# Somedaywilldo/BM-NAS

Measured on AMD Instinct MI355X. Metric: search-steps/sec (fwd+bwd of fusion hypernet) on MM-IMDB synthetic, higher is better.
Workload: dtype f32; 1 GPU; mmimdb fusion search, batch 128 per GPU x 1 GPU(s), N6 C192 L16 steps2 node_steps1 node_multiplier1, train mode, dropout 0.1/0.1(attn); inputs=(b, C, L) features, global_batch=128, per_gpu_batch=128, parallelism=dp1, mode=graph, step=fwd+bwd, one hipGraph replay

## Files before the change

### bm-nas_amd/bmnas/cell.py

```python
from __future__ import annotations

import os

import torch

from . import lib

ATTN_DROP = 0.1

OVERLAP = False
_SIDE = {}


class _Fork:

    def __init__(self, device):
        self.main = torch.cuda.current_stream(device)
        if OVERLAP:
            key = (device.index, self.main.cuda_stream)
            s = _SIDE.get(key)
            if s is None:
                s = torch.cuda.Stream(device)
                _SIDE[key] = s
            self.stream = s
# ... 309 lines not shown
    sv.stats1 = _empty(x, b * 2)
    sv.p1 = p1
    sv.d_glu = DROP.make(P.glu_p, x.numel(), training)
    sv.d_fc = DROP.make(P.fc_p, x.numel(), training)
    sv.merged = same and FUSE_ATTN_GEMM
    if sv.merged:
        U, chan = _mixed_conv_fwd(sv, x, y, same, P, training, C,
                                  attn=(x, y, P.ln_w, P.ln_b, p1, sv.xhat1, sv.stats1, C, sv.d_attn), Weff=Weff,
                                  stats=stats)
    else:
        with _Fork(x.device) as fork:
            fork.side(lambda: lib.sdpa_ln_fwd(x, y, P.ln_w, P.ln_b, p1, sv.xhat1, sv.stats1, b, C, L, sv.d_attn))
            U, chan = _mixed_conv_fwd(sv, x, y, same, P, training, C, Weff=Weff, stats=stats)
    out = torch.empty_like(x)
    fin = sv.conv.fin
    if not launch_mix:
        sv.pending_mix = (x, y, p1, U, chan, gamma_row, out, sv.d_glu, sv.d_fc, fin)
        return out, sv
    if ln is None:
        lib.node_mix_fwd(x, y, p1, U, chan, gamma_row, out, b, C, L, sv.d_glu, sv.d_fc, fin, nxt)
    else:
        resid, ln_w, ln_b, ln_stats, out_sums, lazy = ln
        sv.pre = torch.empty_like(x)
        if lazy:
            P = lib.lazy_ln_parts(C, L)
            rec, prm = _empty(x, b * P * 8), _empty(x, P * 8)
            lib.node_mix_pre_fwd(x, y, p1, U, chan, gamma_row, resid, ln_w, ln_b, sv.pre, rec, prm, b, C, L,
                                 sv.d_glu, sv.d_fc, fin)
            sv.lazy = LazyNode(desc=lib.make_lazy(sv.pre, rec, prm, ln_w, ln_b, ln_stats), out=out, P=P,
                               rec=rec, prm=prm)
        else:
            lib.node_mix_ln_fwd(x, y, p1, U, chan, gamma_row, resid, ln_w, ln_b, sv.pre, out, ln_stats, b, C, L,
                                sv.d_glu, sv.d_fc, fin, out_sums)
    return out, sv


FUSE_ATTN_GEMM = os.environ.get('BMNAS_FUSE_ATTN_GEMM', '1') != '0'
FUSE_PROLOGUE = os.environ.get('BMNAS_FUSE_PROLOGUE', '1') != '0'
FUSE_EPILOGUE = os.environ.get('BMNAS_FUSE_EPILOGUE', '1') != '0'
FUSE_BN_FINALIZE = os.environ.get('BMNAS_FUSE_BN_FINALIZE', '1') != '0'
FUSE_BN_APPLY = os.environ.get('BMNAS_FUSE_BN_APPLY', '1') != '0'
FUSE_MIX_GEMM = os.environ.get('BMNAS_FUSE_MIX_GEMM', '1') != '0'
FUSE_BWD_PAIR = os.environ.get('BMNAS_FUSE_BWD_PAIR', '1') != '0'
FUSE_BN_TAIL = os.environ.get('BMNAS_FUSE_BN_TAIL', '1') != '0'
BN_TAIL_MAX_B = 128
FUSE_INNER_SUM = os.environ.get('BMNAS_FUSE_INNER_SUM', '1') != '0'
MIX_PREV_MAX = 5
FUSE_PROLOGUE_PAIR = os.environ.get('BMNAS_FUSE_PROLOGUE_PAIR', '1') != '0'
FUSE_LN_BWD = os.environ.get('BMNAS_FUSE_LN_BWD', '1') != '0'
FUSE_NEXT_PAIR = os.environ.get('BMNAS_FUSE_NEXT_PAIR', '1') != '0'
FUSE_MIX_EPILOGUE = os.environ.get('BMNAS_FUSE_MIX_EPILOGUE', '1') != '0'
FUSE_HEAD = os.environ.get('BMNAS_FUSE_HEAD', '1') != '0'
LAZY_LN = os.environ.get('BMNAS_LAZY_LN', '1') != '0'
WRITE_ONCE = os.environ.get('BMNAS_WRITE_ONCE', '1') != '0'


STRICT_ZERO = os.environ.get('BMNAS_STRICT_ZERO', '0') not in ('0', '', 'false', 'False')


DETERMINISTIC = os.environ.get('BMNAS_DETERMINISTIC', '0') not in ('0', '', 'false', 'False')
_DET_APPLIED = [None]


def apply_deterministic():
    if _DET_APPLIED[0] != DETERMINISTIC:
        lib.set_deterministic(DETERMINISTIC)
        _DET_APPLIED[0] = DETERMINISTIC


def arch_shards(b, C, L):
    if not DETERMINISTIC:
        return ARCH_SHARDS
    cl4 = C * L // 4
    parts = (cl4 + 255) // 256
    streaming = min(2048, (b * cl4 + 255) // 256)
    mix = ((cl4 + 63) // 64) * lib.node_mix_lnp_bwd_rows(b)
    return max(ARCH_SHARDS, b * parts, streaming, mix)


class LazyNode(Pack):
    materialised = False
    lnp_head = None
    lnp_k1 = None
    k1_n = 0


def _mixed_conv_fwd(sv, x, y, same, P, training, C, attn=None, Weff=None, stats=None):
    if same:
        if Weff is None:
            M = P.stack_W.shape[0]
            Weff = _empty(x, M, C)
            lib.fold_weight(P.stack_W, Weff, M, C)
        U, chan, sv.conv = conv_bn_fwd([x], C, Weff, C, P.stack_bias, P.stack_bn_w, P.stack_bn_b,
                                       P.stack_rm, P.stack_rv, P.stack_nbt, training, dup=C, attn=attn,
                                       stats=stats)
    else:
        U, chan, sv.conv = conv_bn_fwd([x, y], C, P.stack_W, 2 * C, P.stack_bias, P.stack_bn_w,
                                       P.stack_bn_b, P.stack_rm, P.stack_rv, P.stack_nbt, training,
                                       stats=stats)
    return U, chan


class Deferred:

# ... 375 lines not shown

def fusion_cell_fwd(xs, alpha_w, beta_ws, gamma_ws, CP, training, S, M, ns, nm, weffs=None, stats=None,
                    head=None, prologue=None):
    N = len(xs)
    b, C, L = xs[0].shape
    sv = CellSaved()
    sv.N, sv.S, sv.M, sv.CP, sv.alpha_w = N, S, M, CP, alpha_w
    states = list(xs)
    sv.sifs, sv.nodes, sv.offsets = [], [], []
    offset = 0
    pending_pair = None
    sv.lazy_on = bool(LAZY_LN and head is not None and nm == 1 and FUSE_TAIL and FUSE_PAIR and N + S <= 15
                      and 1 <= S <= 3 and M <= S and (C * L) % 64 == 0 and xs[0].is_cuda and lib.lazy_ln_ok(C, L))
    for i in range(S):
        if pending_pair is not None:
            sif, z0 = pending_pair
            pending_pair = None
        elif FUSE_PAIR and len(states) <= 15:
            sif, z0 = torch.empty_like(xs[0]), torch.empty_like(xs[0])
            lz = sv.nodes[-1].lazy if (sv.lazy_on and i >= 1) else None
            if i == 0 and prologue is not None:
                prologue(states, sif, z0)
            elif lz is not None and not lz.materialised:
                lib.mixsum_pair_fwd_lazy(states[:-1], alpha_w[offset:, 1], 2, beta_ws[i][:, 1], 2, lz.desc,
                                         states[-1], sv.nodes[-1].osum, sif, z0, b, C, L)
                lz.materialised = True
            else:
                lib.mixsum_pair_fwd(states, alpha_w[offset:, 1], 2, beta_ws[i][:, 1], 2, sif, z0)
        else:
            sif, z0 = mixsum_fwd(states, alpha_w[offset:, 1]), None
        if STRICT_ZERO:
            if i == 0:
                poison = xs[0] * 0.
                for x_ in xs[1:]:
                    poison = poison + x_ * 0.
            sif.add_(poison)
            if z0 is not None:
                z0.add_(poison)
        next_pair = None
        if (FUSE_NEXT_PAIR and FUSE_PAIR and FUSE_BN_TAIL and i + 1 < S and nm != 1 and len(states) + 1 <= 15
                and lib.bn_relu_ln_fwd_pair_ok(b, C, L, len(states))):
            nsif, nz0 = torch.empty_like(xs[0]), torch.empty_like(xs[0])
            next_pair = (list(states), alpha_w[offset + len(states):, 1], 2, beta_ws[i + 1][:, 1], 2, nsif, nz0)
        out, nsv = node_cell_fwd(sif, sif, beta_ws[i], gamma_ws[i], CP.nodes[i], training, ns, nm, z0,
                                 None if weffs is None else weffs[i * ns:(i + 1) * ns], stats,
                                 want_sums=head is not None, next_pair=next_pair, lazy=sv.lazy_on)
        if next_pair is not None and nsv.next_pair_done:
            pending_pair = (next_pair[5], next_pair[6])
        nsv.paired = z0 is not None
        sv.sifs.append(sif)
        sv.nodes.append(nsv)
        sv.offsets.append(offset)
        offset += len(states)
        states.append(out)
    sv.states = states
    sv.stats = _empty(xs[0], b * 2)
    sv.head = head
    if head is not None:
        if M > S:
            raise lib.BmnasError('fused head: the cell concatenates input states (multiplier > steps)')
        head.sums = [nsv.osum for nsv in sv.nodes[S - M:]]
        if DETERMINISTIC and (not sv.lazy_on or ns != 1):
            raise lib.BmnasError('BMNAS_DETERMINISTIC covers the search cell with node_steps == 1 and node_multiplier '
                                 '== 1 under the fused head (the lazy-LayerNorm path); this configuration is outside it')
        last = sv.nodes[-1].lazy if sv.lazy_on else None
        if last is not None and not last.materialised:
            O_ = head.W.shape[0]
            hb_part = _empty(xs[0], lib.head_fwd_part_floats(b, C, L, M, O_)) if DETERMINISTIC else None
            lib.head_fwd_lazy(states[-M:-1] + [sv.nodes[-1].o], head.sums[:-1] + [None], M - 1, last.desc, CP.ln_w,
# ... 162 lines not shown
```

### bm-nas_amd/bmnas/lib.py

```python
import ctypes as C
import os

import torch

HERE = os.path.dirname(os.path.abspath(__file__))
LIB_PATH = os.environ.get('BMNAS_LIB') or os.path.join(HERE, 'libbmnas_hip.so')
MAX_PTRS = 16


class BmnasError(RuntimeError):
    pass


_NOTED = set()


def note_off_path(where, why):
    key = (where, why)
    if key not in _NOTED:
        _NOTED.add(key)
        import warnings
        warnings.warn(f'bmnas: {where} runs on the stock torch ops, not the HIP kernels: {why}', RuntimeWarning,
                      stacklevel=3)

# ... 205 lines not shown
    'bmnas_unroll_virtual_step': ([_P, _P, _I, _P, _I, _P], _I),
    'bmnas_unroll_perturb': ([_P, _P, _I, _P, _I, _P, C.c_float, _P, _P], _I),
    'bmnas_unroll_restore': ([_P, _P, _I, _P], _I),
    'bmnas_unroll_combine': ([_P, _P, _I, _P, _P, _P], _I),
    'bmnas_copy_batch_max': ([], _I),
    'bmnas_copy_blob_max': ([], _I),
    'bmnas_copy_batch': ([_PP, _PP, C.POINTER(C.c_longlong), _I, _P, _P, _I, _P, C.c_ulonglong, _P], _I),
    'bmnas_arch_softmax_fwd': ([_P, _P, _I, _I, _P], _I),
    'bmnas_arch_softmax_bwd': ([_P, _P, _P, _I, _I, _P], _I),
    'bmnas_backward_epilogue': ([_I, _PP, _PP, C.POINTER(_PP), C.POINTER(C.c_int), _PP, _PP, _PP, _PP, _PP,
                                 _PP, _I, C.POINTER(C.c_int), _I, C.POINTER(C.c_int), C.POINTER(C.c_int),
                                 _PP, _PP, _PP, C.POINTER(C.c_int), C.POINTER(C.c_int), _I, _I, _I64,
                                 _I, _PP, _PP, C.POINTER(C.c_int), C.POINTER(C.c_int64), _P], _I),
    'bmnas_head_chunks': ([_I], _I),
    'bmnas_head_fwd': ([_PP, _PP, _I, _P, _P, _P, _P, _P, _P, _I, _I, _I, _I, _P], _I),
    'bmnas_debug_stamps': ([_P, _I], _I),
    'bmnas_debug_stamps_head': ([_P, _I], _I),
    'bmnas_debug_stamps_conv': ([_P, _I], _I),
    'bmnas_lazy_ln_ok': ([_I, _I], _I),
    'bmnas_lazy_ln_parts': ([_I, _I], _I),
    'bmnas_node_mix_pre_fwd': ([_P, _P, _P, _P, _P, BnFin, _P, _P, _P, _P, _P, _P, _P, _I, _I, _I, Dropout, Dropout,
                                _P], _I),
    'bmnas_mixsum_pair_fwd_lazy': ([_PP, _I, _P, _I, _P, _I, C.POINTER(LazyLn), _P, _P, _P, _P, _I, _I, _I, _P], _I),
    'bmnas_mixsum_pair_bwd_lazy': ([_PP, _PP, _I, _P, _I, _P, _I, _P, _P, _P, _P, _P, _P, _I, _I64, _U32,
                                    C.POINTER(LazyLn), _PP, C.POINTER(C.c_int), _I, _P, _I, _I, _I, _P], _I),
    'bmnas_mixsum_pair_bwd_x': ([_PP, _PP, _I, _P, _I, _P, _I, _P, _P, _P, _P, _P, _P, _I, _I64, _U32, _PP, _PP, _I,
                                 _I64, _P], _I),
    'bmnas_head_fwd_lazy': ([_PP, _PP, _I, _I, C.POINTER(LazyLn), _P, _P, _P, _P, _P, _P, _I, _I, _I, _I, _P, _P], _I),
    'bmnas_head_fwd_part_floats': ([_I, _I, _I, _I, _I], _I),
    'bmnas_node_mix_lnp_bwd_rows': ([_I], _I),
    'bmnas_conv1x1_set_deterministic': ([_I], _I),
    'bmnas_ln_set_deterministic': ([_I], _I),
    'bmnas_head_bwd_lazy': ([C.POINTER(LazyLn), _PP, _PP, _I, _U32, _P, _P, _P, _P, _P, _I, _P, _P, _P, _P, _P,
                             _I, _I, _I, _I, _P, _I64, _P, _P], _I),
    'bmnas_node_mix_lnp_bwd': ([_P, _P, _P, _P, _P, _I, _P, _I, _P, _P, _I, _P, _P, _P, _P, _P, _P, _P, _I, _I64,
                                _P, _P, _U32, _P, _P, _I, _I, _I, Dropout, Dropout, _P, _P], _I),
    'bmnas_head_bwd': ([_PP, _PP, _PP, _I, _U32, _P, _P, _P, _P, _P, _I, _P, _P, _P, _P, _P, _I, _I, _I, _I,
                        _P, _I64, _P], _I),
    'bmnas_head_bwd_crit': ([_PP, _PP, _PP, _I, _U32, _P, _P, _P, _P, _P, _I, _P, _P, _P, _P, _I, _I, _I, _I,
                             _P, _I64, CriterionDesc, _P], _I),
    'bmnas_head_bwd_lazy_crit': ([C.POINTER(LazyLn), _PP, _PP, _I, _U32, _P, _P, _P, _P, _P, _I, _P, _P, _P, _P,
                                  _I, _I, _I, _I, _P, _I64, _P, CriterionDesc, _P], _I),
    'bmnas_bce_logits_crit': ([_P, _P, CriterionDesc, _P, _P, _I, _I, _P], _I),
    'bmnas_cross_entropy_crit': ([_P, _P, CriterionDesc, _P, _P, _P, _I, _I, _P], _I),
    'bmnas_sum_chunks': ([_P, _P, _I, _I64, _P], _I),
    'bmnas_comm_available': ([], _I),
# ... 224 lines not shown


def lazy_ln_ok(Cc, L):
    return bool(load().bmnas_lazy_ln_ok(Cc, L))


def lazy_ln_parts(Cc, L):
    n = load().bmnas_lazy_ln_parts(Cc, L)
    if n < 1:
        _check(n, 'lazy_ln_parts')
    return n


def make_lazy(pre, rec, prm, ln_w, ln_b, stats):
    return LazyLn(_ptr(pre), _ptr(rec), _ptr(prm), _ptr(ln_w), _ptr(ln_b), _ptr(stats))


def node_mix_pre_fwd(x, y, p1, U, chan, gamma, resid, ln_w, ln_b, pre, rec, prm, b, Cc, L, dglu, dfc, fin=NO_FIN):
    _check(load().bmnas_node_mix_pre_fwd(_ptr(x), _ptr(y), _ptr(p1), _ptr(U), _ptr(chan), fin, gamma.data_ptr(),
                                         _ptr(resid), _ptr(ln_w), _ptr(ln_b), _ptr(pre), _ptr(rec), _ptr(prm),
                                         b, Cc, L, dglu, dfc, _stream()), 'node_mix_pre_fwd')


def mixsum_pair_fwd_lazy(xs, w, w_stride, w2, w2_stride, lazy, last_out, last_sums, out, out2, b, Cc, L):
    _check(load().bmnas_mixsum_pair_fwd_lazy(_ptrs(xs), len(xs), w.data_ptr(), w_stride, w2.data_ptr(), w2_stride,
                                             C.byref(lazy), _ptr(last_out), _ptr(last_sums), _ptr(out), _ptr(out2),
                                             b, Cc, L, _stream()), 'mixsum_pair_fwd_lazy')


def mixsum_pair_bwd_lazy(xs, dxs, w, w_stride, w2, w2_stride, h, gh, gz, dw, dw2, acc_mask, lazies, lnparts, strides,
                         b, Cc, L, dw_shards=1, dw_shard_stride=0, gz2=None, g_full=None):
    n = len(lazies)
    arr = (LazyLn * n)(*lazies)
    st = (C.c_int * n)(*strides)
    _check(load().bmnas_mixsum_pair_bwd_lazy(_ptrs(xs), _ptrs(dxs), len(xs), w.data_ptr(), w_stride, w2.data_ptr(),
                                             w2_stride, _ptr(h), _ptr(gh), _ptr(gz), _ptr(gz2), _opt(dw),
                                             _opt(dw2), dw_shards, dw_shard_stride, acc_mask, arr,
                                             (C.c_void_p * n)(*[t.data_ptr() for t in lnparts]), st, n,
                                             _ptr(g_full), b, Cc, L, _stream()),
           'mixsum_pair_bwd_lazy')


def mixsum_pair_bwd_x(xs, dxs, w, w_stride, w2, w2_stride, h, gh, gz, dw, dw2, acc_mask, g_more, w_more, dw_shards=1,
                      dw_shard_stride=0, gz2=None):
    n = len(g_more)
    _check(load().bmnas_mixsum_pair_bwd_x(_ptrs(xs), _ptrs(dxs), len(xs), w.data_ptr(), w_stride, w2.data_ptr(),
                                          w2_stride, _ptr(h), _ptr(gh), _ptr(gz), _ptr(gz2), _opt(dw),
# ... 852 lines not shown
```

### bm-nas_amd/csrc/lazyln.hip

```cpp
#include "common.hpp"
#include "../../include/bmnas_hip.h"
#include "bn_fin.hpp"
#include "lazy_ln.hpp"
#include "mix_common.hpp"

namespace {

__global__ __launch_bounds__(256) void node_mix_pre_fwd_k(
    const float* __restrict__ x, const float* __restrict__ y, const float* __restrict__ p1,
    const float* __restrict__ U, float* __restrict__ chan, BnFin fin, const float* __restrict__ gamma,
    const float* __restrict__ resid, const float* __restrict__ ln_w, const float* __restrict__ ln_b,
    float* __restrict__ pre, float* __restrict__ rec, float* __restrict__ prm, int b, int C, int L,
    DropCfg dglu, DropCfg dfc) {
  __shared__ float red[4];
  __shared__ float red5[2 * 4 * 5];
  extern __shared__ float fin_lds[];
  const int cl4 = C * L / 4, l4n = L / 4, M = 3 * C;
  const int part = blockIdx.x, smp = blockIdx.y, P = gridDim.x;
  STAMP(0, smp * P + part, 0);
  float* sc = fin_lds;
  float* sh = fin_lds + M;
  const int r0 = part * kLazyPart + threadIdx.x;
  const bool act = r0 < cl4;
  const int r = act ? r0 : cl4 - 1;
  const int c = r / l4n;
  const int64_t e = ((int64_t)smp * cl4 + r) * 4;
  const int64_t ub = ((int64_t)smp * M) * L + (int64_t)r * 4;
  const float4 lw = ld4(ln_w + (int64_t)r * 4), lb = ld4(ln_b + (int64_t)r * 4);
  const float4 ua = ld4(U + ub), ug = ld4(U + ub + (int64_t)C * L), uf = ld4(U + ub + (int64_t)2 * C * L);
  const float4 xv = ld4(x + e), yv = ld4(y + e), pv = ld4(p1 + e), rv = ld4(resid + e);
  __builtin_amdgcn_sched_barrier(0);
  const float g0 = gamma[0], g1 = gamma[1], g2 = gamma[2], g3 = gamma[3];
  const DropRt rglu = drop_begin(dglu), rfc = drop_begin(dfc);
  STAMP(0, smp * P + part, 1);
  bn_fin_fill<256>(fin, chan, M, b * L, sc, sh, part == 0 && smp == 0);
  STAMP(0, smp * P + part, 2);
  const float4 va = affine4(ua, sc[c], sh[c]);
  const float4 vg = affine4(ug, sc[C + c], sh[C + c]);
  const float4 vf = affine4(uf, sc[2 * C + c], sh[2 * C + c]);
  const float4 m2 = drop_mult4(rglu, (uint64_t)e), m3 = drop_mult4(rfc, (uint64_t)e);
  const float4 o = mix_fwd4<kMixAll>(g0, g1, g2, g3, f4_add(xv, yv), pv, va, vg, vf, m2, m3);
  const float4 v = f4_add(o, rv);
  if (act) st4_w0<3>(pre + e, v);
  STAMP(0, smp * P + part, 3);
  const int n4 = cl4 - part * kLazyPart < kLazyPart ? cl4 - part * kLazyPart : kLazyPart;
  const float nk = (float)(4 * n4);
  float mk = wave_sum(act ? f4_hsum(v) : 0.f);
  const int wv = threadIdx.x >> 6, ln = threadIdx.x & 63;
  if (ln == 0) red[wv] = mk;
  __syncthreads();
  mk = (((red[0] + red[1]) + red[2]) + red[3]) / nk;
  float acc[5] = {0.f, 0.f, 0.f, 0.f, 0.f};
  if (act) {
    const float4 cd = make_float4(v.x - mk, v.y - mk, v.z - mk, v.w - mk);
    const float4 cw = f4_mul(cd, lw);
    acc[0] = f4_dot(cd, cd);
    acc[1] = f4_hsum(cw);
    acc[2] = f4_dot(cw, cw);
    acc[3] = f4_dot(cw, lb);
    acc[4] = f4_dot(cw, lw);
  }
  float pa[5] = {0.f, 0.f, 0.f, 0.f, 0.f};
  if (smp == 0 && act) {
    pa[0] = f4_dot(lw, lw);
    pa[1] = f4_hsum(lw);
    pa[2] = f4_dot(lw, lb);
    pa[3] = f4_hsum(lb);
    pa[4] = f4_dot(lb, lb);
  }
#pragma unroll
  for (int i = 0; i < 5; ++i) acc[i] = wave_sum(acc[i]);
  if (smp == 0) {
#pragma unroll
    for (int i = 0; i < 5; ++i) pa[i] = wave_sum(pa[i]);
  }
  if (ln == 0) {
#pragma unroll
    for (int i = 0; i < 5; ++i) red5[i * 4 + wv] = acc[i];
    if (smp == 0) {
#pragma unroll
      for (int i = 0; i < 5; ++i) red5[20 + i * 4 + wv] = pa[i];
    }
  }
  __syncthreads();
  if (threadIdx.x == 0) {
    float t[5];
#pragma unroll
    for (int i = 0; i < 5; ++i) t[i] = ((red5[i * 4] + red5[i * 4 + 1]) + red5[i * 4 + 2]) + red5[i * 4 + 3];
    float* rr = rec + ((int64_t)smp * P + part) * kLazyRec;
    st4(rr, make_float4(mk, t[0], t[1], t[2]));
    st4(rr + 4, make_float4(t[3], t[4], 0.f, 0.f));
  }
  STAMP(0, smp * P + part, 4);
  if (smp == 0 && threadIdx.x == 64) {
    float t[5];
#pragma unroll
    for (int i = 0; i < 5; ++i)
      t[i] = ((red5[20 + i * 4] + red5[20 + i * 4 + 1]) + red5[20 + i * 4 + 2]) + red5[20 + i * 4 + 3];
    st4(prm + part * kLazyRec, make_float4(t[0], t[1], t[2], t[3]));
    st4(prm + part * kLazyRec + 4, make_float4(t[4], nk, 0.f, 0.f));
  }
}

template <int NIN>
__global__ __launch_bounds__(256) void mixsum_pair_fwd_lazy_k(
    PtrsIn xs, const float* __restrict__ w, int w_stride, const float* __restrict__ w2, int w2_stride,
    const float* __restrict__ pre, const float* __restrict__ rec, const float* __restrict__ prm,
    const float* __restrict__ ln_w, const float* __restrict__ ln_b, float* __restrict__ nout,
    float* __restrict__ stats, float* __restrict__ osum, float* __restrict__ out, float* __restrict__ out2,
    int cl4) {
  const int part = blockIdx.x, smp = blockIdx.y, P = gridDim.x;
  STAMP(1, smp * P + part, 0);
  const int r0 = part * kLazyPart + threadIdx.x;
  const bool act = r0 < cl4;
  const int r = act ? r0 : cl4 - 1;
  const int64_t i = (int64_t)smp * cl4 + r;
  float wj[NIN + 1];
#pragma unroll
  for (int j = 0; j <= NIN; ++j) wj[j] = w[j * w_stride];
  const float s2 = w2[0] + w2[w2_stride];
  float4 v[NIN];
#pragma unroll
  for (int j = 0; j < NIN; ++j) v[j] = reinterpret_cast<const float4*>(xs.p[j])[i];
  const float4 pv = reinterpret_cast<const float4*>(pre)[i];
  const float4 lw = ld4(ln_w + (int64_t)r * 4), lb = ld4(ln_b + (int64_t)r * 4);
  const LazyStats st = lazy_combine(rec, prm, P, smp);
  const float4 n = make_float4((pv.x - st.mean) * st.rstd * lw.x + lb.x, (pv.y - st.mean) * st.rstd * lw.y + lb.y,
                               (pv.z - st.mean) * st.rstd * lw.z + lb.z, (pv.w - st.mean) * st.rstd * lw.w + lb.w);
  float4 acc = f4_scale(v[0], wj[0]);
#pragma unroll
  for (int j = 1; j < NIN; ++j) {
    acc.x = fmaf(wj[j], v[j].x, acc.x);
    acc.y = fmaf(wj[j], v[j].y, acc.y);
    acc.z = fmaf(wj[j], v[j].z, acc.z);
    acc.w = fmaf(wj[j], v[j].w, acc.w);
  }
  acc.x = fmaf(wj[NIN], n.x, acc.x);
  acc.y = fmaf(wj[NIN], n.y, acc.y);
  acc.z = fmaf(wj[NIN], n.z, acc.z);
  acc.w = fmaf(wj[NIN], n.w, acc.w);
  if (act) {
    st4_w0<4>(nout + 4 * i, n);
    st4_w0<4>(out + 4 * i, acc);
    st4_w0<4>(out2 + 4 * i, f4_scale(acc, s2));
  }
  STAMP(1, smp * P + part, 1);
  if (part == 0 && threadIdx.x == 0) {
    stats[2 * smp] = st.mean;
    stats[2 * smp + 1] = st.rstd;
    if (osum != nullptr) {
      osum[2 * smp] = st.osum;
      osum[2 * smp + 1] = st.osq;
    }
  }
}

constexpr int kMaxLazyIn = 2;
struct LazyIn {
  const float* pre[kMaxLazyIn];
  const float* ln_w[kMaxLazyIn];
  const float* stats[kMaxLazyIn];
  float* lnpart[kMaxLazyIn];
  int stride[kMaxLazyIn];
};

template <int NIN, int NLZ, bool DOTS = true>
__global__ __launch_bounds__(256) void mixsum_pair_bwd_lazy_k(
    PtrsIn xs, PtrsOut dxs, const float* __restrict__ w, int w_stride, const float* __restrict__ w2, int w2_stride,
    const float* __restrict__ h, const float* __restrict__ gh, const float* __restrict__ gz,
    const float* __restrict__ gz2, float* dw, float* dw2, int dw_shards, int64_t dw_shard_stride, uint32_t acc_mask,
// ... 330 lines not shown
    if (!xs[j]) return BMNAS_E_ARG;
    p.p[j] = xs[j];
  }
  const int cl4 = C * L / 4;
  dim3 grid(lazy_parts(cl4), b);
  hipStream_t st = (hipStream_t)stream;
#define CALL(N)                                                                                              \
  hipLaunchKernelGGL(mixsum_pair_fwd_lazy_k<N>, grid, dim3(256), 0, st, p, w, w_stride, w2, w2_stride,       \
                     last->pre, last->rec, last->prm, last->ln_w, last->ln_b, last_out, last->stats,         \
                     last_sums, out, out2, cl4)
  switch (n_in) {
    case 1: CALL(1); break;   case 2: CALL(2); break;   case 3: CALL(3); break;
    case 4: CALL(4); break;   case 5: CALL(5); break;   case 6: CALL(6); break;
    case 7: CALL(7); break;   case 8: CALL(8); break;   case 9: CALL(9); break;
    case 10: CALL(10); break; case 11: CALL(11); break; case 12: CALL(12); break;
    case 13: CALL(13); break; case 14: CALL(14); break; case 15: CALL(15); break;
    default: return BMNAS_E_LIMIT;
  }
#undef CALL
  BMNAS_CHECK_LAUNCH();
  return 0;
}

extern "C" int bmnas_mixsum_pair_bwd_lazy(const float* const* xs, float* const* dxs, int n_in, const float* w,
                                          int w_stride, const float* w2, int w2_stride, const float* h,
                                          const float* gh, const float* gz, const float* gz2, float* dw, float* dw2,
                                          int dw_shards, int64_t dw_shard_stride, uint32_t accumulate_mask,
                                          const bmnas_lazy_ln_t* lazy, float* const* lnpart,
                                          const int* lnpart_stride, int n_lazy, float* g_full, int b, int C, int L,
                                          void* stream) {
  if (!xs || !dxs || !w || !w2 || !h || !gz || !lazy || !lnpart || !lnpart_stride || n_in < 1 || b < 0 ||
      w_stride < 1 || w2_stride < 1 || dw_shards < 1)
    return BMNAS_E_ARG;
  if ((dw == nullptr) != (dw2 == nullptr)) return BMNAS_E_ARG;
  const bool dots = dw != nullptr;
  if (n_lazy < 1 || n_lazy > kMaxLazyIn || n_lazy >= n_in) return BMNAS_E_LIMIT;
  if (n_in > BMNAS_MAX_PTRS - 1) return BMNAS_E_LIMIT;
  if (!bmnas_lazy_ln_ok(C, L)) return BMNAS_E_LIMIT;
  if (b == 0) return 0;
  PtrsIn p{};
  PtrsOut d{};
  for (int j = 0; j < n_in; ++j) {
    if (!xs[j]) return BMNAS_E_ARG;
    p.p[j] = xs[j];
    d.p[j] = dxs[j];
  }
// ... 89 lines not shown
```

### include/bmnas_hip.h

```cpp
#ifndef BMNAS_HIP_H
#define BMNAS_HIP_H

#include <stdint.h>

#ifdef __cplusplus
extern "C" {
#endif

#define BMNAS_MAX_PTRS 16
#define BMNAS_E_ARG (-1)
#define BMNAS_E_SHAPE (-2)
#define BMNAS_E_LIMIT (-3)

typedef struct {
  uint32_t thr;
  float scale;
  uint64_t seed;
  uint64_t offset;
  const uint64_t* step;
} bmnas_dropout_t;

int bmnas_version(void);

int bmnas_dropout_mask(bmnas_dropout_t drop, int64_t n_elem, float* out, void* stream);
// ... 306 lines not shown
                   uint32_t accumulate_mask, const float* ln_w, const float* ln_b, const float* W,
                   const float* hb, const float* stats, int mode, const float* g, const float* gscale,
                   const void* labels, float* loss, float* part, int b, int C, int L, int O, float* scrub,
                   int64_t scrub_n, void* stream);
int bmnas_sum_chunks(const float* part, float* out, int n_chunk, int64_t n, void* stream);

typedef struct {
  const float* pre;
  const float* rec;
  const float* prm;
  const float* ln_w;
  const float* ln_b;
  float* stats;
} bmnas_lazy_ln_t;
int bmnas_lazy_ln_ok(int C, int L);
int bmnas_lazy_ln_parts(int C, int L);
int bmnas_node_mix_pre_fwd(const float* x, const float* y, const float* p1, const float* U, float* chan,
                           bmnas_bn_fin_t fin, const float* gamma, const float* resid, const float* ln_w,
                           const float* ln_b, float* pre, float* rec, float* prm, int b, int C, int L,
                           bmnas_dropout_t drop_glu, bmnas_dropout_t drop_fc, void* stream);
int bmnas_mixsum_pair_fwd_lazy(const float* const* xs, int n_in, const float* w, int w_stride, const float* w2,
                               int w2_stride, const bmnas_lazy_ln_t* last, float* last_out, float* last_sums,
                               float* out, float* out2, int b, int C, int L, void* stream);
int bmnas_mixsum_pair_bwd_lazy(const float* const* xs, float* const* dxs, int n_in, const float* w, int w_stride,
                               const float* w2, int w2_stride, const float* h, const float* gh, const float* gz,
                               const float* gz2, float* dw, float* dw2, int dw_shards, int64_t dw_shard_stride,
                               uint32_t accumulate_mask, const bmnas_lazy_ln_t* lazy, float* const* lnpart,
                               const int* lnpart_stride, int n_lazy, float* g_full, int b, int C, int L,
                               void* stream);
int bmnas_mixsum_pair_bwd_x(const float* const* xs, float* const* dxs, int n_in, const float* w, int w_stride,
                            const float* w2, int w2_stride, const float* h, const float* gh, const float* gz,
                            const float* gz2, float* dw, float* dw2, int dw_shards, int64_t dw_shard_stride,
                            uint32_t accumulate_mask, const float* const* g_more, const float* const* w_more,
                            int n_more, int64_t n_elem, void* stream);
int bmnas_head_fwd_lazy(const float* const* srcs, const float* const* sums, int n_src, int lazy_q,
                        const bmnas_lazy_ln_t* lazy, const float* ln_w, const float* ln_b, const float* W,
                        const float* bias, float* hb, float* stats, int b, int C, int L, int O, float* hb_part,
                        void* stream);
int bmnas_head_bwd_lazy(const bmnas_lazy_ln_t* lazy, float* const* lnpart, float* const* dsrcs, int n_src,
                        uint32_t accumulate_mask, const float* ln_w, const float* ln_b, const float* W,
                        const float* hb, const float* stats, int mode, const float* g, const float* gscale,
                        const void* labels, float* loss, float* part, int b, int C, int L, int O, float* scrub,
                        int64_t scrub_n, float* loss_part, void* stream);
int bmnas_node_mix_lnp_bwd(const float* g, const float* pre, const float* ln_w, const float* stats,
                           const float* lnp0, int n0, const float* lnp1, int n1, float* g_in, float* dresid,
                           int accumulate_resid, const float* x, const float* y, const float* p1, const float* U,
// ... 180 lines not shown
```

Before: 7401 steps/s.

## Fuse node mix pre-LN kernel with next step's lazy-LN pair sum

```diff
diff --git a/bm-nas_amd/bmnas/cell.py b/bm-nas_amd/bmnas/cell.py
--- a/bm-nas_amd/bmnas/cell.py
+++ b/bm-nas_amd/bmnas/cell.py
@@ -355,7 +355,12 @@
     else:
         resid, ln_w, ln_b, ln_stats, out_sums, lazy = ln
         sv.pre = torch.empty_like(x)
-        if lazy:
+        if lazy == 'pair':
+            pend = lib.PendingMixPre(x, y, p1, U, chan, gamma_row, resid, ln_w, ln_b, sv.pre, ln_stats, sv.d_glu,
+                                     sv.d_fc, fin)
+            sv.lazy = LazyNode(desc=pend.desc, out=out, P=lib.lazy_ln_parts(C, L), rec=None, prm=None,
+                               pending_mix=pend)
+        elif lazy:
             P = lib.lazy_ln_parts(C, L)
             rec, prm = _empty(x, b * P * 8), _empty(x, P * 8)
             lib.node_mix_pre_fwd(x, y, p1, U, chan, gamma_row, resid, ln_w, ln_b, sv.pre, rec, prm, b, C, L,
@@ -386,6 +391,7 @@
 FUSE_HEAD = os.environ.get('BMNAS_FUSE_HEAD', '1') != '0'
 LAZY_LN = os.environ.get('BMNAS_LAZY_LN', '1') != '0'
 WRITE_ONCE = os.environ.get('BMNAS_WRITE_ONCE', '1') != '0'
+FUSE_MIX_PAIR = os.environ.get('BMNAS_FUSE_MIX_PAIR', '1') != '0'
 
 
 STRICT_ZERO = os.environ.get('BMNAS_STRICT_ZERO', '0') not in ('0', '', 'false', 'False')
@@ -413,6 +419,7 @@
 
 class LazyNode(Pack):
     materialised = False
+    pending_mix = None
     lnp_head = None
     lnp_k1 = None
     k1_n = 0
@@ -834,13 +841,16 @@
             if i == 0 and prologue is not None:
                 prologue(states, sif, z0)
             elif lz is not None and not lz.materialised:
-                lib.mixsum_pair_fwd_lazy(states[:-1], alpha_w[offset:, 1], 2, beta_ws[i][:, 1], 2, lz.desc,
+                lib.mixsum_pair_fwd_lazy(states[:-1], alpha_w[offset:, 1], 2, beta_ws[i][:, 1], 2,
+                                         lz.pending_mix if lz.pending_mix is not None else lz.desc,
                                          states[-1], sv.nodes[-1].osum, sif, z0, b, C, L)
                 lz.materialised = True
             else:
                 lib.mixsum_pair_fwd(states, alpha_w[offset:, 1], 2, beta_ws[i][:, 1], 2, sif, z0)
         else:
             sif, z0 = mixsum_fwd(states, alpha_w[offset:, 1]), None
+        if i >= 1 and getattr(sv.nodes[-1].lazy, 'pending_mix', None) is not None and not sv.nodes[-1].lazy.materialised:
+            raise lib.BmnasError('a step node left its mix to the next K1 pair sum, which did not take it')
         if STRICT_ZERO:
             if i == 0:
                 poison = xs[0] * 0.
@@ -854,9 +864,12 @@
                 and lib.bn_relu_ln_fwd_pair_ok(b, C, L, len(states))):
             nsif, nz0 = torch.empty_like(xs[0]), torch.empty_like(xs[0])
             next_pair = (list(states), alpha_w[offset + len(states):, 1], 2, beta_ws[i + 1][:, 1], 2, nsif, nz0)
+        mix_pair = (sv.lazy_on and FUSE_MIX_PAIR and i + 1 < S
+                    and lib.node_mix_pair_fwd_lazy_ok(b, C, L, len(states)))
         out, nsv = node_cell_fwd(sif, sif, beta_ws[i], gamma_ws[i], CP.nodes[i], training, ns, nm, z0,
                                  None if weffs is None else weffs[i * ns:(i + 1) * ns], stats,
-                                 want_sums=head is not None, next_pair=next_pair, lazy=sv.lazy_on)
+                                 want_sums=head is not None, next_pair=next_pair,
+                                 lazy='pair' if mix_pair else sv.lazy_on)
         if next_pair is not None and nsv.next_pair_done:
             pending_pair = (next_pair[5], next_pair[6])
         nsv.paired = z0 is not None
diff --git a/bm-nas_amd/bmnas/lib.py b/bm-nas_amd/bmnas/lib.py
--- a/bm-nas_amd/bmnas/lib.py
+++ b/bm-nas_amd/bmnas/lib.py
@@ -251,6 +251,9 @@
     'bmnas_node_mix_pre_fwd': ([_P, _P, _P, _P, _P, BnFin, _P, _P, _P, _P, _P, _P, _P, _I, _I, _I, Dropout, Dropout,
                                 _P], _I),
     'bmnas_mixsum_pair_fwd_lazy': ([_PP, _I, _P, _I, _P, _I, C.POINTER(LazyLn), _P, _P, _P, _P, _I, _I, _I, _P], _I),
+    'bmnas_node_mix_pair_fwd_lazy_ok': ([_I, _I, _I, _I], _I),
+    'bmnas_node_mix_pair_fwd_lazy': ([_P, _P, _P, _P, _P, BnFin, _P, _P, _P, _P, _P, _I, _I, _I, Dropout, Dropout,
+                                      _PP, _I, _P, _I, _P, _I, _P, _P, _P, _P, _P, _P], _I),
     'bmnas_mixsum_pair_bwd_lazy': ([_PP, _PP, _I, _P, _I, _P, _I, _P, _P, _P, _P, _P, _P, _I, _I64, _U32,
                                     C.POINTER(LazyLn), _PP, C.POINTER(C.c_int), _I, _P, _I, _I, _I, _P], _I),
     'bmnas_mixsum_pair_bwd_x': ([_PP, _PP, _I, _P, _I, _P, _I, _P, _P, _P, _P, _P, _P, _I, _I64, _U32, _PP, _PP, _I,
@@ -521,7 +524,27 @@
                                          b, Cc, L, dglu, dfc, _stream()), 'node_mix_pre_fwd')
 
 
+def node_mix_pair_fwd_lazy_ok(b, Cc, L, n_in):
+    return bool(load().bmnas_node_mix_pair_fwd_lazy_ok(int(b), int(Cc), int(L), int(n_in)))
+
+
+class PendingMixPre:
+
+    def __init__(self, x, y, p1, U, chan, gamma, resid, ln_w, ln_b, pre, stats, dglu, dfc, fin):
+        self.x, self.y, self.p1, self.U, self.chan, self.gamma, self.resid = x, y, p1, U, chan, gamma, resid
+        self.ln_w, self.ln_b, self.pre, self.stats, self.dglu, self.dfc, self.fin = ln_w, ln_b, pre, stats, dglu, dfc, fin
+        self.desc = make_lazy(pre, None, None, ln_w, ln_b, stats)
+
+
 def mixsum_pair_fwd_lazy(xs, w, w_stride, w2, w2_stride, lazy, last_out, last_sums, out, out2, b, Cc, L):
+    if isinstance(lazy, PendingMixPre):
+        m = lazy
+        _check(load().bmnas_node_mix_pair_fwd_lazy(
+            _ptr(m.x), _ptr(m.y), _ptr(m.p1), _ptr(m.U), _ptr(m.chan), m.fin, m.gamma.data_ptr(), _ptr(m.resid),
+            _ptr(m.ln_w), _ptr(m.ln_b), _ptr(m.pre), b, Cc, L, m.dglu, m.dfc, _ptrs(xs), len(xs), w.data_ptr(),
+            w_stride, w2.data_ptr(), w2_stride, _ptr(last_out), _ptr(last_sums), _ptr(m.stats), _ptr(out), _ptr(out2),
+            _stream()), 'node_mix_pair_fwd_lazy')
+        return
     _check(load().bmnas_mixsum_pair_fwd_lazy(_ptrs(xs), len(xs), w.data_ptr(), w_stride, w2.data_ptr(), w2_stride,
                                              C.byref(lazy), _ptr(last_out), _ptr(last_sums), _ptr(out), _ptr(out2),
                                              b, Cc, L, _stream()), 'mixsum_pair_fwd_lazy')
diff --git a/bm-nas_amd/csrc/lazyln.hip b/bm-nas_amd/csrc/lazyln.hip
--- a/bm-nas_amd/csrc/lazyln.hip
+++ b/bm-nas_amd/csrc/lazyln.hip
@@ -5,6 +5,76 @@
 #include "mix_common.hpp"
 
 namespace {
+
+struct PreOps {
+  float4 lw, lb, ua, ug, uf, xv, yv, pv, rv;
+};
+
+__device__ __forceinline__ PreOps pre_loads(const float* __restrict__ x, const float* __restrict__ y,
+                                            const float* __restrict__ p1, const float* __restrict__ U,
+                                            const float* __restrict__ resid, const float* __restrict__ ln_w,
+                                            const float* __restrict__ ln_b, const int r, const int64_t e,
+                                            const int64_t ub, const int C, const int L) {
+  PreOps o;
+  o.lw = ld4(ln_w + (int64_t)r * 4), o.lb = ld4(ln_b + (int64_t)r * 4);
+  o.ua = ld4(U + ub), o.ug = ld4(U + ub + (int64_t)C * L), o.uf = ld4(U + ub + (int64_t)2 * C * L);
+  o.xv = ld4(x + e), o.yv = ld4(y + e), o.pv = ld4(p1 + e), o.rv = ld4(resid + e);
+  return o;
+}
+
+__device__ __forceinline__ float4 pre_value(const PreOps& o, const float* sc, const float* sh, const int c, const int C,
+                                            const float g0, const float g1, const float g2, const float g3,
+                                            const DropRt& rglu, const DropRt& rfc, const int64_t e) {
+  const float4 va = affine4(o.ua, sc[c], sh[c]);
+  const float4 vg = affine4(o.ug, sc[C + c], sh[C + c]);
+  const float4 vf = affine4(o.uf, sc[2 * C + c], sh[2 * C + c]);
+  const float4 m2 = drop_mult4(rglu, (uint64_t)e), m3 = drop_mult4(rfc, (uint64_t)e);
+  const float4 m = mix_fwd4<kMixAll>(g0, g1, g2, g3, f4_add(o.xv, o.yv), o.pv, va, vg, vf, m2, m3);
+  return f4_add(m, o.rv);
+}
+
+__device__ __forceinline__ void pre_centred(const float4 v, const float mk, const float4 lw, const float4 lb,
+                                            float (&acc)[5]) {
+  const float4 cd = make_float4(v.x - mk, v.y - mk, v.z - mk, v.w - mk);
+  const float4 cw = f4_mul(cd, lw);
+  acc[0] = f4_dot(cd, cd);
+  acc[1] = f4_hsum(cw);
+  acc[2] = f4_dot(cw, cw);
+  acc[3] = f4_dot(cw, lb);
+  acc[4] = f4_dot(cw, lw);
+}
+
+__device__ __forceinline__ void pre_affine(const float4 lw, const float4 lb, float (&pa)[5]) {
+  pa[0] = f4_dot(lw, lw);
+  pa[1] = f4_hsum(lw);
+  pa[2] = f4_dot(lw, lb);
+  pa[3] = f4_hsum(lb);
+  pa[4] = f4_dot(lb, lb);
+}
+
+__device__ __forceinline__ float sum4w(const float* q) { return ((q[0] + q[1]) + q[2]) + q[3]; }
+
+__device__ __forceinline__ float4 lazy_norm4(const float4 pv, const LazyStats& st, const float4 lw, const float4 lb) {
+  return make_float4((pv.x - st.mean) * st.rstd * lw.x + lb.x, (pv.y - st.mean) * st.rstd * lw.y + lb.y,
+                     (pv.z - st.mean) * st.rstd * lw.z + lb.z, (pv.w - st.mean) * st.rstd * lw.w + lb.w);
+}
+
+template <int NIN>
+__device__ __forceinline__ float4 pair_sum(const float4 (&v)[NIN], const float (&wj)[NIN + 1], const float4 n) {
+  float4 acc = f4_scale(v[0], wj[0]);
+#pragma unroll
+  for (int j = 1; j < NIN; ++j) {
+    acc.x = fmaf(wj[j], v[j].x, acc.x);
+    acc.y = fmaf(wj[j], v[j].y, acc.y);
+    acc.z = fmaf(wj[j], v[j].z, acc.z);
+    acc.w = fmaf(wj[j], v[j].w, acc.w);
+  }
+  acc.x = fmaf(wj[NIN], n.x, acc.x);
+  acc.y = fmaf(wj[NIN], n.y, acc.y);
+  acc.z = fmaf(wj[NIN], n.z, acc.z);
+  acc.w = fmaf(wj[NIN], n.w, acc.w);
+  return acc;
+}
 
 __global__ __launch_bounds__(256) void node_mix_pre_fwd_k(
     const float* __restrict__ x, const float* __restrict__ y, const float* __restrict__ p1,
@@ -26,21 +96,15 @@
   const int c = r / l4n;
   const int64_t e = ((int64_t)smp * cl4 + r) * 4;
   const int64_t ub = ((int64_t)smp * M) * L + (int64_t)r * 4;
-  const float4 lw = ld4(ln_w + (int64_t)r * 4), lb = ld4(ln_b + (int64_t)r * 4);
-  const float4 ua = ld4(U + ub), ug = ld4(U + ub + (int64_t)C * L), uf = ld4(U + ub + (int64_t)2 * C * L);
-  const float4 xv = ld4(x + e), yv = ld4(y + e), pv = ld4(p1 + e), rv = ld4(resid + e);
+  const PreOps o = pre_loads(x, y, p1, U, resid, ln_w, ln_b, r, e, ub, C, L);
+  const float4 lw = o.lw, lb = o.lb;
   __builtin_amdgcn_sched_barrier(0);
   const float g0 = gamma[0], g1 = gamma[1], g2 = gamma[2], g3 = gamma[3];
   const DropRt rglu = drop_begin(dglu), rfc = drop_begin(dfc);
   STAMP(0, smp * P + part, 1);
   bn_fin_fill<256>(fin, chan, M, b * L, sc, sh, part == 0 && smp == 0);
   STAMP(0, smp * P + part, 2);
-  const float4 va = affine4(ua, sc[c], sh[c]);
-  const float4 vg = affine4(ug, sc[C + c], sh[C + c]);
-  const float4 vf = affine4(uf, sc[2 * C + c], sh[2 * C + c]);
-  const float4 m2 = drop_mult4(rglu, (uint64_t)e), m3 = drop_mult4(rfc, (uint64_t)e);
-  const float4 o = mix_fwd4<kMixAll>(g0, g1, g2, g3, f4_add(xv, yv), pv, va, vg, vf, m2, m3);
-  const float4 v = f4_add(o, rv);
+  const float4 v = pre_value(o, sc, sh, c, C, g0, g1, g2, g3, rglu, rfc, e);
   if (act) st4_w0<3>(pre + e, v);
   STAMP(0, smp * P + part, 3);
   const int n4 = cl4 - part * kLazyPart < kLazyPart ? cl4 - part * kLazyPart : kLazyPart;
@@ -49,25 +113,11 @@
   const int wv = threadIdx.x >> 6, ln = threadIdx.x & 63;
   if (ln == 0) red[wv] = mk;
   __syncthreads();
-  mk = (((red[0] + red[1]) + red[2]) + red[3]) / nk;
+  mk = sum4w(red) / nk;
   float acc[5] = {0.f, 0.f, 0.f, 0.f, 0.f};
-  if (act) {
-    const float4 cd = make_float4(v.x - mk, v.y - mk, v.z - mk, v.w - mk);
-    const float4 cw = f4_mul(cd, lw);
-    acc[0] = f4_dot(cd, cd);
-    acc[1] = f4_hsum(cw);
-    acc[2] = f4_dot(cw, cw);
-    acc[3] = f4_dot(cw, lb);
-    acc[4] = f4_dot(cw, lw);
-  }
+  if (act) pre_centred(v, mk, lw, lb, acc);
   float pa[5] = {0.f, 0.f, 0.f, 0.f, 0.f};
-  if (smp == 0 && act) {
-    pa[0] = f4_dot(lw, lw);
-    pa[1] = f4_hsum(lw);
-    pa[2] = f4_dot(lw, lb);
-    pa[3] = f4_hsum(lb);
-    pa[4] = f4_dot(lb, lb);
-  }
+  if (smp == 0 && act) pre_affine(lw, lb, pa);
 #pragma unroll
   for (int i = 0; i < 5; ++i) acc[i] = wave_sum(acc[i]);
   if (smp == 0) {
@@ -86,7 +136,7 @@
   if (threadIdx.x == 0) {
     float t[5];
 #pragma unroll
-    for (int i = 0; i < 5; ++i) t[i] = ((red5[i * 4] + red5[i * 4 + 1]) + red5[i * 4 + 2]) + red5[i * 4 + 3];
+    for (int i = 0; i < 5; ++i) t[i] = sum4w(red5 + i * 4);
     float* rr = rec + ((int64_t)smp * P + part) * kLazyRec;
     st4(rr, make_float4(mk, t[0], t[1], t[2]));
     st4(rr + 4, make_float4(t[3], t[4], 0.f, 0.f));
@@ -95,8 +145,7 @@
   if (smp == 0 && threadIdx.x == 64) {
     float t[5];
 #pragma unroll
-    for (int i = 0; i < 5; ++i)
-      t[i] = ((red5[20 + i * 4] + red5[20 + i * 4 + 1]) + red5[20 + i * 4 + 2]) + red5[20 + i * 4 + 3];
+    for (int i = 0; i < 5; ++i) t[i] = sum4w(red5 + 20 + i * 4);
     st4(prm + part * kLazyRec, make_float4(t[0], t[1], t[2], t[3]));
     st4(prm + part * kLazyRec + 4, make_float4(t[4], nk, 0.f, 0.f));
   }
@@ -125,20 +174,8 @@
   const float4 pv = reinterpret_cast<const float4*>(pre)[i];
   const float4 lw = ld4(ln_w + (int64_t)r * 4), lb = ld4(ln_b + (int64_t)r * 4);
   const LazyStats st = lazy_combine(rec, prm, P, smp);
-  const float4 n = make_float4((pv.x - st.mean) * st.rstd * lw.x + lb.x, (pv.y - st.mean) * st.rstd * lw.y + lb.y,
-                               (pv.z - st.mean) * st.rstd * lw.z + lb.z, (pv.w - st.mean) * st.rstd * lw.w + lb.w);
-  float4 acc = f4_scale(v[0], wj[0]);
-#pragma unroll
-  for (int j = 1; j < NIN; ++j) {
-    acc.x = fmaf(wj[j], v[j].x, acc.x);
-    acc.y = fmaf(wj[j], v[j].y, acc.y);
-    acc.z = fmaf(wj[j], v[j].z, acc.z);
-    acc.w = fmaf(wj[j], v[j].w, acc.w);
-  }
-  acc.x = fmaf(wj[NIN], n.x, acc.x);
-  acc.y = fmaf(wj[NIN], n.y, acc.y);
-  acc.z = fmaf(wj[NIN], n.z, acc.z);
-  acc.w = fmaf(wj[NIN], n.w, acc.w);
+  const float4 n = lazy_norm4(pv, st, lw, lb);
+  const float4 acc = pair_sum<NIN>(v, wj, n);
   if (act) {
     st4_w0<4>(nout + 4 * i, n);
     st4_w0<4>(out + 4 * i, acc);
@@ -146,6 +183,113 @@
   }
   STAMP(1, smp * P + part, 1);
   if (part == 0 && threadIdx.x == 0) {
+    stats[2 * smp] = st.mean;
+    stats[2 * smp + 1] = st.rstd;
+    if (osum != nullptr) {
+      osum[2 * smp] = st.osum;
+      osum[2 * smp + 1] = st.osq;
+    }
+  }
+}
+
+#ifndef BMNAS_MIX_PAIR_K1_EARLY
+#define BMNAS_MIX_PAIR_K1_EARLY 0
+#endif
+template <int NIN, int P>
+__global__ __launch_bounds__(256 * P) void node_mixsum_pair_fwd_lazy_k(
+    const float* __restrict__ x, const float* __restrict__ y, const float* __restrict__ p1,
+    const float* __restrict__ U, float* __restrict__ chan, BnFin fin, const float* __restrict__ gamma,
+    const float* __restrict__ resid, const float* __restrict__ ln_w, const float* __restrict__ ln_b,
+    float* __restrict__ pre, int b, int C, int L, DropCfg dglu, DropCfg dfc, PtrsIn xs,
+    const float* __restrict__ w, int w_stride, const float* __restrict__ w2, int w2_stride,
+    float* __restrict__ nout, float* __restrict__ stats, float* __restrict__ osum, float* __restrict__ out,
+    float* __restrict__ out2) {
+  __shared__ float red[P * 4];
+  __shared__ float red5[P * 2 * 4 * 5];
+  __shared__ __attribute__((aligned(16))) float recs[P * kLazyRec];
+  __shared__ __attribute__((aligned(16))) float prms[P * kLazyRec];
+  extern __shared__ float fin_lds[];
+  const int cl4 = C * L / 4, l4n = L / 4, M = 3 * C;
+  const int part = threadIdx.x >> 8, tp = threadIdx.x & 255, smp = blockIdx.x;
+  float* sc = fin_lds;
+  float* sh = fin_lds + M;
+  const int r0 = part * kLazyPart + tp;
+  const bool act = r0 < cl4;
+  const int r = act ? r0 : cl4 - 1;
+  const int c = r / l4n;
+  const int64_t i = (int64_t)smp * cl4 + r;
+  const int64_t e = i * 4;
+  const int64_t ub = ((int64_t)smp * M) * L + (int64_t)r * 4;
+  const PreOps o = pre_loads(x, y, p1, U, resid, ln_w, ln_b, r, e, ub, C, L);
+  const float4 lw = o.lw, lb = o.lb;
+  float4 xv[NIN];
+#if BMNAS_MIX_PAIR_K1_EARLY
+#pragma unroll
+  for (int j = 0; j < NIN; ++j) xv[j] = reinterpret_cast<const float4*>(xs.p[j])[i];
+#endif
+  __builtin_amdgcn_sched_barrier(0);
+  const float g0 = gamma[0], g1 = gamma[1], g2 = gamma[2], g3 = gamma[3];
+  const DropRt rglu = drop_begin(dglu), rfc = drop_begin(dfc);
+  float wj[NIN + 1];
+#pragma unroll
+  for (int j = 0; j <= NIN; ++j) wj[j] = w[j * w_stride];
+  const float s2 = w2[0] + w2[w2_stride];
+  bn_fin_fill<256 * P>(fin, chan, M, b * L, sc, sh, smp == 0);
+  const float4 v = pre_value(o, sc, sh, c, C, g0, g1, g2, g3, rglu, rfc, e);
+  if (act) st4_w0<3>(pre + e, v);
+#if !BMNAS_MIX_PAIR_K1_EARLY
+#pragma unroll
+  for (int j = 0; j < NIN; ++j) xv[j] = reinterpret_cast<const float4*>(xs.p[j])[i];
+#endif
+  const int n4 = cl4 - part * kLazyPart < kLazyPart ? cl4 - part * kLazyPart : kLazyPart;
+  const float nk = (float)(4 * n4);
+  float mk = wave_sum(act ? f4_hsum(v) : 0.f);
+  const int wv = tp >> 6, ln = tp & 63;
+  if (ln == 0) red[part * 4 + wv] = mk;
+  __syncthreads();
+  mk = sum4w(red + part * 4) / nk;
+  float acc[5] = {0.f, 0.f, 0.f, 0.f, 0.f};
+  if (act) pre_centred(v, mk, lw, lb, acc);
+  float pa[5] = {0.f, 0.f, 0.f, 0.f, 0.f};
+  if (act) pre_affine(lw, lb, pa);
+#pragma unroll
+  for (int q = 0; q < 5; ++q) acc[q] = wave_sum(acc[q]);
+#pragma unroll
+  for (int q = 0; q < 5; ++q) pa[q] = wave_sum(pa[q]);
+  float* r5 = red5 + part * 40;
+  if (ln == 0) {
+#pragma unroll
+    for (int q = 0; q < 5; ++q) r5[q * 4 + wv] = acc[q];
+#pragma unroll
+    for (int q = 0; q < 5; ++q) r5[20 + q * 4 + wv] = pa[q];
+  }
+  __syncthreads();
+  if (tp == 0) {
+    float t[5];
+#pragma unroll
+    for (int q = 0; q < 5; ++q) t[q] = sum4w(r5 + q * 4);
+    st4(recs + part * kLazyRec, make_float4(mk, t[0], t[1], t[2]));
+    st4(recs + part * kLazyRec + 4, make_float4(t[3], t[4], 0.f, 0.f));
+  }
+  if (tp == 64) {
+    float t[5];
+#pragma unroll
+    for (int q = 0; q < 5; ++q) t[q] = sum4w(r5 + 20 + q * 4);
+    st4(prms + part * kLazyRec, make_float4(t[0], t[1], t[2], t[3]));
+    st4(prms + part * kLazyRec + 4, make_float4(t[4], nk, 0.f, 0.f));
+  }
+  __syncthreads();
+  int Pr = P;
+  asm volatile("" : "+s"(Pr));
+  const LazyStats st = lazy_combine(recs, prms, Pr, 0);
+  const float4 n = lazy_norm4(v, st, lw, lb);
+  const float4 h = pair_sum<NIN>(xv, wj, n);
+  if (act) {
+    st4_w0<4>(nout + e, n);
+    st4_w0<4>(out + e, h);
+    st4_w0<4>(out2 + e, f4_scale(h, s2));
+  }
+  if (threadIdx.x == 0) {
     stats[2 * smp] = st.mean;
     stats[2 * smp + 1] = st.rstd;
     if (osum != nullptr) {
@@ -522,6 +666,91 @@
   return 0;
 }
 
+constexpr int kMixPairMaxIn = 14;
+constexpr int kMixPairMaxIn3 = 10;
+constexpr int kMixPairMaxP = 3;
+
+extern "C" int bmnas_node_mix_pair_fwd_lazy_ok(int b, int C, int L, int n_in) {
+  if (b < 1 || n_in < 1 || n_in > kMixPairMaxIn || !bmnas_lazy_ln_ok(C, L)) return 0;
+  if (C > 4096 / 3 || (3 * C) % 4) return 0;
+  const int P = lazy_parts(C * L / 4);
+  return P <= kMixPairMaxP && n_in <= (P == 3 ? kMixPairMaxIn3 : kMixPairMaxIn);
+}
+
+namespace {
+struct MixPairArgs {
+  const float *x, *y, *p1, *U;
+  float* chan;
+  BnFin f;
+  const float *gamma, *resid, *ln_w, *ln_b;
+  float* pre;
+  int b, C, L;
+  DropCfg dglu, dfc;
+  PtrsIn xs;
+  const float* w;
+  int w_stride;
+  const float* w2;
+  int w2_stride;
+  float *nout, *stats, *osum, *out, *out2;
+  hipStream_t st;
+};
+
+template <int P>
+int launch_mix_pair(const MixPairArgs& a, int n_in) {
+#define CALL(N)                                                                                                   \
+  hipLaunchKernelGGL((node_mixsum_pair_fwd_lazy_k<N, P>), dim3(a.b), dim3(256 * P), (size_t)6 * a.C * sizeof(float), \
+                     a.st, a.x, a.y, a.p1, a.U, a.chan, a.f, a.gamma, a.resid, a.ln_w, a.ln_b, a.pre, a.b, a.C, a.L, \
+                     a.dglu, a.dfc, a.xs, a.w, a.w_stride, a.w2, a.w2_stride, a.nout, a.stats, a.osum, a.out, a.out2)
+  switch (n_in) {
+    case 1: CALL(1); break;   case 2: CALL(2); break;   case 3: CALL(3); break;
+    case 4: CALL(4); break;   case 5: CALL(5); break;   case 6: CALL(6); break;
+    case 7: CALL(7); break;   case 8: CALL(8); break;   case 9: CALL(9); break;
+    case 10: CALL(10); break; case 11: CALL(11); break; case 12: CALL(12); break;
+    case 13: CALL(13); break; case 14: CALL(14); break;
+    default: return BMNAS_E_LIMIT;
+  }
+#undef CALL
+  BMNAS_CHECK_LAUNCH();
+  return 0;
+}
+}
+
+extern "C" int bmnas_node_mix_pair_fwd_lazy(const float* x, const float* y, const float* p1, const float* U,
+                                            float* chan, bmnas_bn_fin_t fin, const float* gamma, const float* resid,
+                                            const float* ln_w, const float* ln_b, float* pre, int b, int C, int L,
+                                            bmnas_dropout_t drop_glu, bmnas_dropout_t drop_fc,
+                                            const float* const* xs, int n_in, const float* w, int w_stride,
+                                            const float* w2, int w2_stride, float* last_out, float* last_sums,
+                                            float* stats, float* out, float* out2, void* stream) {
+  if (!x || !y || !p1 || !U || !chan || !gamma || !resid || !ln_w || !ln_b || !pre || b < 0 || C < 1)
+    return BMNAS_E_ARG;
+  if (!xs || !w || !w2 || !stats || !last_out || !out || !out2 || n_in < 1 || w_stride < 1 || w2_stride < 1)
+    return BMNAS_E_ARG;
+  if (!(L == 4 || L == 8 || L == 16)) return BMNAS_E_SHAPE;
+  if (n_in > BMNAS_MAX_PTRS - 1) return BMNAS_E_LIMIT;
+  if (!bmnas_lazy_ln_ok(C, L)) return BMNAS_E_LIMIT;
+  MixPairArgs a{};
+  if (int e = to_fin(fin, &a.f)) return e;
+  if (a.f.on && a.f.training && b * L < 2) return BMNAS_E_ARG;
+  if (C > 4096 / 3 || (3 * C) % 4) return BMNAS_E_LIMIT;
+  if (b == 0) return 0;
+  for (int j = 0; j < n_in; ++j) {
+    if (!xs[j]) return BMNAS_E_ARG;
+    a.xs.p[j] = xs[j];
+  }
+  if (!bmnas_node_mix_pair_fwd_lazy_ok(b, C, L, n_in)) return BMNAS_E_LIMIT;
+  a.x = x; a.y = y; a.p1 = p1; a.U = U; a.chan = chan; a.gamma = gamma; a.resid = resid; a.ln_w = ln_w; a.ln_b = ln_b;
+  a.pre = pre; a.b = b; a.C = C; a.L = L; a.dglu = to_cfg(drop_glu); a.dfc = to_cfg(drop_fc);
+  a.w = w; a.w_stride = w_stride; a.w2 = w2; a.w2_stride = w2_stride;
+  a.nout = last_out; a.stats = stats; a.osum = last_sums; a.out = out; a.out2 = out2; a.st = (hipStream_t)stream;
+  switch (lazy_parts(C * L / 4)) {
+    case 1: return launch_mix_pair<1>(a, n_in);
+    case 2: return launch_mix_pair<2>(a, n_in);
+    case 3: return launch_mix_pair<3>(a, n_in);
+    default: return BMNAS_E_LIMIT;
+  }
+}
+
 extern "C" int bmnas_mixsum_pair_bwd_lazy(const float* const* xs, float* const* dxs, int n_in, const float* w,
                                           int w_stride, const float* w2, int w2_stride, const float* h,
                                           const float* gh, const float* gz, const float* gz2, float* dw, float* dw2,
diff --git a/include/bmnas_hip.h b/include/bmnas_hip.h
--- a/include/bmnas_hip.h
+++ b/include/bmnas_hip.h
@@ -352,6 +352,13 @@
 int bmnas_mixsum_pair_fwd_lazy(const float* const* xs, int n_in, const float* w, int w_stride, const float* w2,
                                int w2_stride, const bmnas_lazy_ln_t* last, float* last_out, float* last_sums,
                                float* out, float* out2, int b, int C, int L, void* stream);
+int bmnas_node_mix_pair_fwd_lazy_ok(int b, int C, int L, int n_in);
+int bmnas_node_mix_pair_fwd_lazy(const float* x, const float* y, const float* p1, const float* U, float* chan,
+                                 bmnas_bn_fin_t fin, const float* gamma, const float* resid, const float* ln_w,
+                                 const float* ln_b, float* pre, int b, int C, int L, bmnas_dropout_t drop_glu,
+                                 bmnas_dropout_t drop_fc, const float* const* xs, int n_in, const float* w,
+                                 int w_stride, const float* w2, int w2_stride, float* last_out, float* last_sums,
+                                 float* stats, float* out, float* out2, void* stream);
 int bmnas_mixsum_pair_bwd_lazy(const float* const* xs, float* const* dxs, int n_in, const float* w, int w_stride,
                                const float* w2, int w2_stride, const float* h, const float* gh, const float* gz,
                                const float* gz2, float* dw, float* dw2, int dw_shards, int64_t dw_shard_stride,
```

After: 7437 steps/s, median of 6. About the same (+0.5%).
